# orting/image-feature-extraction

Hardware: AMD Instinct MI355X
Metric: Mvoxels/sec Hessian+eig, 512^3 fp32 3-scale (higher is better)
Workload: dtype f32 storage / f64 line recurrences

## Files before the change

image-feature-extraction_amd/__init__.py:

```python
import ctypes as C
import os

import numpy as np

_HERE = os.path.dirname(os.path.abspath(__file__))
LIB_PATH = os.environ.get("IFE_HIP_LIB") or os.path.join(_HERE, "csrc", "libife_hip.so")

OK, E_ARG, E_SIZE, E_HIP, E_NOMEM, E_STATE = 0, -1, -2, -3, -4, -5
F32, I16, U8, U16 = 0, 1, 2, 3
INTERLEAVED, PLANAR = 0, 1
MEM_HOST, MEM_DEVICE = 0, 1
OPT_TRIG_MODE, OPT_DSCALE_MODE, OPT_PROFILE, OPT_ZCHUNK, OPT_IIR_BLOCK, OPT_IIR_CKPT, OPT_IIR_FMA = 1, 2, 3, 4, 5, 6, 7
OPT_FUSED_DIVIDE = 8
OPT_CONST_LINES = 9
OPT_FEAT_RING = 10
Z_STATE_BYTES = 32
Z_OVERLAP_LO, Z_OVERLAP_HI = 3, 4
NUM_FEATURES = 8
MAX_KERNEL_KINDS = 24
FEATURE_NAMES = ("GaussianBlur", "GradientMagnitude", "Eigenvalue1", "Eigenvalue2",
                 "Eigenvalue3", "LaplacianOfGaussian", "GaussianCurvature", "FrobeniusNorm")

EXPORTS = (
    "ife_abi_version", "ife_ctx_create", "ife_ctx_destroy", "ife_last_error",
    "ife_ctx_set_stream", "ife_ctx_set_option", "ife_ctx_reserve", "ife_ctx_synchronize",
    "ife_eigenvalues", "ife_eigenvalue_features", "ife_hessian3d", "ife_gradient_magnitude",
    "ife_normalized_gaussian_convolution", "ife_differential_normalized_convolution",
    "ife_emphysema_features",
    "ife_emphysema_features_begin", "ife_emphysema_features_fetch", "ife_emphysema_features_end",
    "ife_fd_hessian_features", "ife_fd_gradient_features", "ife_mask_image_f64",
    "ife_get_kernel_times", "ife_reset_kernel_times", "ife_measure_stream",
    "ife_stage_prepare", "ife_stage_recursive_gaussian", "ife_stage_recursive_gaussian_batch",
    "ife_stage_features", "ife_stage_z_ck_bytes", "ife_stage_z_sweep", "ife_stage_z_combine",
    "ife_stage_z_fused", "ife_stage_recursive_gaussian_quotient",
    "ife_multi_create", "ife_multi_destroy", "ife_multi_last_error", "ife_multi_set_option",
    "ife_multi_emphysema_features", "ife_multi_emphysema_features_begin",
    "ife_multi_emphysema_features_fetch", "ife_multi_emphysema_features_end",
    "ife_sort_f32", "ife_equalized_edges_f32", "ife_equalized_edges_f64", "ife_dense_histogram_f32", "ife_roi_histograms", "ife_bag_image",
    "ife_samples_create", "ife_samples_destroy", "ife_samples_count", "ife_samples_clear",
    "ife_samples_add_features", "ife_samples_add_image", "ife_samples_sort",
    "ife_samples_equalized_edges", "ife_samples_read_column",
    "ife_signed_distance_map", "ife_expected_distance",
)


class VolumeDesc(C.Structure):
    _fields_ = [("nx", C.c_int64), ("ny", C.c_int64), ("nz", C.c_int64),
                ("sx", C.c_double), ("sy", C.c_double), ("sz", C.c_double)]
# ... 642 lines not shown
```

image-feature-extraction_amd/csrc/eigen_device.hpp:

```cpp
#pragma once
#include <hip/hip_runtime.h>

namespace ife {

struct Eig3 {
  float e0, e1, e2;
};

template <int TRIG>
__device__ __forceinline__ Eig3 eig3_sym(float A11, float A12, float A13, float A22, float A23,
                                         float A33) {
  Eig3 r;
  float p = A12 * A12 + A13 * A13 + A23 * A23;
  if (p == 0.0f) {
    const float a1 = fabsf(A11), a2 = fabsf(A22), a3 = fabsf(A33);
    if (a1 > a2) {
      if (a1 > a3) {
        r.e0 = A11;
        if (a2 > a3) { r.e1 = A22; r.e2 = A33; }
        else         { r.e1 = A33; r.e2 = A22; }
      } else { r.e0 = A33; r.e1 = A11; r.e2 = A22; }
    } else {
      if (a2 > a3) {
        r.e0 = A22;
// ... 218 lines not shown
    r.e0 = diag ? d0 : r.e0;
    r.e1 = diag ? d1 : r.e1;
    r.e2 = diag ? d2 : r.e2;
  }
  if (__builtin_amdgcn_ballot_w64(unsafe) != 0) {
    const Eig3 g = eig3_sym_generic_call<(TRIG == 2 ? 0 : TRIG)>(A11, A12, A13, A22, A23, A33);
    r.e0 = unsafe ? g.e0 : r.e0;
    r.e1 = unsafe ? g.e1 : r.e1;
    r.e2 = unsafe ? g.e2 : r.e2;
  }
  return r;
}

__device__ __forceinline__ float sqrt_rn_normal(float x) {
  const float s = __builtin_amdgcn_sqrtf(x);
  const float sd = __builtin_bit_cast(float, __builtin_bit_cast(int, s) - 1);
  const float su = __builtin_bit_cast(float, __builtin_bit_cast(int, s) + 1);
  const float ed = fmaf(-sd, s, x);
  const float eu = fmaf(-su, s, x);
  float r = ed <= 0.0f ? sd : s;
  r = eu > 0.0f ? su : r;
  return r;
}
template <int D>
__device__ __forceinline__ float div_by_const_inrange(float x) {
  const float d = (float)D;
  const float y = D == 3 ? 0x1.555556p-2f : 0x1.555556p-3f;
  const float q = x * y;
  const float f = fmaf(fmaf(-d, q, x), y, q);
  return x == 0.0f ? x : f;
}

template <typename KT>
__device__ __forceinline__ Eig3 eig3_sym_fast2(float A11, float A12, float A13, float A22,
                                              float A23, float A33, const KT &K) {
  const float p0 = A12 * A12 + A13 * A13 + A23 * A23;
  const bool diag = p0 == 0.0f;
  const float tr = A11 + A22 + A33;
  const float q = div_by_const_inrange<3>(tr);
  const float d1 = A11 - q, d2 = A22 - q, d3 = A33 - q;
  const float p2 = d1 * d1 + d2 * d2 + d3 * d3 + 2.0f * p0;
  const float atr = fabsf(tr);
  const bool ok = (atr <= 0x1p100f) && (atr >= 0x1p-100f || atr == 0.0f) && (p2 >= 0x1p-100f) &&
                  (p2 <= 0x1p100f);
  const bool unsafe = !diag && !ok;
  const float p = sqrt_rn_normal(div_by_const_inrange<6>(p2));
  const SharedRecip rp = shared_recip(p);
  const float B11 = div_shared(d1, rp), B12 = div_shared(A12, rp), B13 = div_shared(A13, rp);
  const float B22 = div_shared(d2, rp), B23 = div_shared(A23, rp), B33 = div_shared(d3, rp);
  const float r2 = B11 * B22 * B33 + 2.0f * B12 * B13 * B23 - B23 * B23 * B11 -
                   B13 * B13 * B22 - B12 * B12 * B33;
  const float rr = r2 * 0.5f;
  const float twop = 2.0f * p;
  float phi = acos_third_f32(rr);
  phi = rr >= 1.0f ? 0.0f : phi;
  phi = rr <= -1.0f ? (float)(M_PI / 3) : phi;
  float e0 = fmaf(twop, cos_small_f32(phi), q);
  float e2 = fmaf(-twop, cos_small_f32((float)(M_PI / 3) - phi), q);
  float e1 = 3.0f * q - e0 - e2;
  if (fabsf(e0) < fabsf(e2)) { const float t = e0; e0 = e2; e2 = t; }
  if (fabsf(e1) < fabsf(e2)) { const float t = e1; e1 = e2; e2 = t; }
  Eig3 r;
  r.e0 = e0; r.e1 = e1; r.e2 = e2;
  if (__builtin_amdgcn_ballot_w64(diag || unsafe) != 0) {
    const float a1 = fabsf(A11), a2 = fabsf(A22), a3 = fabsf(A33);
    const bool c12 = a1 > a2, c13 = a1 > a3, c23 = a2 > a3;
    const float g0 = c12 ? (c13 ? A11 : A33) : (c23 ? A22 : A33);
    const float g1 = c12 ? (c13 ? (c23 ? A22 : A33) : A11) : (c23 ? (c13 ? A11 : A33) : A22);
    const float g2 = c12 ? (c13 ? (c23 ? A33 : A22) : A22) : (c23 ? (c13 ? A33 : A11) : A11);
    r.e0 = diag ? g0 : r.e0;
    r.e1 = diag ? g1 : r.e1;
    r.e2 = diag ? g2 : r.e2;
    if (__builtin_amdgcn_ballot_w64(unsafe) != 0) {
      const Eig3 g = eig3_sym_generic_call<0>(A11, A12, A13, A22, A23, A33);
      r.e0 = unsafe ? g.e0 : r.e0;
      r.e1 = unsafe ? g.e1 : r.e1;
      r.e2 = unsafe ? g.e2 : r.e2;
    }
  }
  return r;
}

struct EigFeat {
  float f[6];
};

template <int TRIG, typename KT = EigConstImm>
__device__ __forceinline__ EigFeat eig_features(float A11, float A12, float A13, float A22,
                                                float A23, float A33, const KT &K = KT()) {
  Eig3 ev;
  if constexpr (TRIG == 2) ev = eig3_sym_fast2(A11, A12, A13, A22, A23, A33, K);
  else ev = eig3_sym_fast<TRIG>(A11, A12, A13, A22, A23, A33, K);
  EigFeat o;
  o.f[0] = ev.e0;
  o.f[1] = ev.e1;
  o.f[2] = ev.e2;
  o.f[3] = ev.e0 + ev.e1 + ev.e2;
  o.f[4] = ev.e0 * ev.e1 * ev.e2;
  o.f[5] = sqrtf(ev.e0 * ev.e0 + ev.e1 * ev.e1 + ev.e2 * ev.e2);
  return o;
}

}
```

image-feature-extraction_amd/csrc/feature_kernels.hpp:

```cpp
#pragma once
#include <hip/hip_runtime.h>
#include <float.h>
#include <stdint.h>

#include "eigen_device.hpp"

namespace ife {

enum FeatMode {
  FEAT_FEATURES8 = 0,
  FEAT_EIG6 = 1,
  FEAT_HESSIAN6 = 2,
  FEAT_GRADMAG = 3,
  FEAT_SAMPLES8 = 4
};

template <int MODE>
struct FeatNOut {
  static constexpr int value =
      (MODE == FEAT_FEATURES8 || MODE == FEAT_SAMPLES8) ? 8 : (MODE == FEAT_GRADMAG ? 1 : 6);
};

struct FeatGeom {
  int nx, ny, nz;
// ... 26 lines not shown
    if (__builtin_amdgcn_ballot_w64(r.b != 1.0f) == 0) return r.a;
    return r.b != 0.0f ? r.a / r.b : FLT_MAX;
  }
};
struct ValS {
  const float *s;
  struct Raw { float a; };
  __device__ __forceinline__ Raw fetch(int64_t i) const { return Raw{s[i]}; }
  __device__ __forceinline__ float finish(const Raw &r) const { return r.a; }
};
template <typename TI>
struct ValRaw {
  const TI *img;
  struct Raw { TI v; };
  __device__ __forceinline__ Raw fetch(int64_t i) const { return Raw{img[i]}; }
  __device__ __forceinline__ float finish(const Raw &r) const { return (float)r.v; }
};

__device__ __forceinline__ int clampi(int v, int hi) { return v < 0 ? 0 : (v > hi ? hi : v); }

__device__ __forceinline__ double d1(double cm, double cp, float fm, float fp) {
  double s = 0.0;
  s += cm * (double)fm;
  s += cp * (double)fp;
  return s;
}
__device__ __forceinline__ float d2(double ca, double cb, double cc, float fm, float f0,
                                    float fp) {
  double s = 0.0;
  s += ca * (double)fm;
  s += cb * (double)f0;
  s += cc * (double)fp;
  return (float)s;
}

constexpr int FT_TX = 64;
#ifndef IFE_FT_TY
#define IFE_FT_TY 8
#endif
constexpr int FT_TY = IFE_FT_TY;
constexpr int FT_HX = FT_TX + 2;
constexpr int FT_HY = FT_TY + 2;
constexpr int FT_NE = FT_HX * FT_HY;
constexpr int FT_THREADS = FT_TX * FT_TY;
constexpr int FT_NLD = (FT_NE + FT_THREADS - 1) / FT_THREADS;

template <int MODE, bool UNIT, int TRIG, bool KLDS>
__device__ __forceinline__ void feat_point(const float (*tm)[FT_HX], const float (*t0)[FT_HX],
                                           const float (*tp)[FT_HX], int ty, int tx,
                                           const DerivCoef &dc, const double *ktab,
                                           float (&o)[FeatNOut<MODE>::value]) {
  constexpr bool F8 = MODE == FEAT_FEATURES8 || MODE == FEAT_SAMPLES8;
  constexpr bool NEED_H = MODE != FEAT_GRADMAG;
  constexpr bool NEED_G = F8 || MODE == FEAT_GRADMAG;
  const float c = t0[ty + 1][tx + 1];
  const float xm = t0[ty + 1][tx], xp = t0[ty + 1][tx + 2];
  const float ym = t0[ty][tx + 1], yp = t0[ty + 2][tx + 1];
  const float zm = tm[ty + 1][tx + 1], zp = tp[ty + 1][tx + 1];
  float G = 0.0f;
  if (NEED_G) {
    double gx, gy, gz;
    if (UNIT) {
      gx = 0.5 * ((double)xp - (double)xm);
      gy = 0.5 * ((double)yp - (double)ym);
      gz = 0.5 * ((double)zp - (double)zm);
    } else {
      gx = d1(dc.m1[0], dc.p1[0], xm, xp);
      gy = d1(dc.m1[1], dc.p1[1], ym, yp);
      gz = d1(dc.m1[2], dc.p1[2], zm, zp);
    }
    double a = gx * gx;
    a += gy * gy;
    a += gz * gz;
#if defined(IFE_DIAG_NO_GSQRT)
    G = (float)a;
#else
    G = (float)sqrt(a);
#endif
  }
  if constexpr (MODE == FEAT_GRADMAG) {
    o[0] = G;
  } else if (NEED_H) {
    const float cmm = t0[ty][tx], cpm = t0[ty][tx + 2];
    const float cmp = t0[ty + 2][tx], cpp = t0[ty + 2][tx + 2];
    const float zm_xm = tm[ty + 1][tx], zm_xp = tm[ty + 1][tx + 2];
    const float zm_ym = tm[ty][tx + 1], zm_yp = tm[ty + 2][tx + 1];
    const float zp_xm = tp[ty + 1][tx], zp_xp = tp[ty + 1][tx + 2];
    const float zp_ym = tp[ty][tx + 1], zp_yp = tp[ty + 2][tx + 1];
    float dxx, dyy, dzz, dxy, dxz, dyz;
    if (UNIT) {
      const float dx_ym = 0.5f * (cpm - cmm), dx_yp = 0.5f * (cpp - cmp);
      const float dx_zm = 0.5f * (zm_xp - zm_xm), dx_zp = 0.5f * (zp_xp - zp_xm);
      const float dy_zm = 0.5f * (zm_yp - zm_ym), dy_zp = 0.5f * (zp_yp - zp_ym);
      dxy = 0.5f * (dx_yp - dx_ym);
      dxz = 0.5f * (dx_zp - dx_zm);
      dyz = 0.5f * (dy_zp - dy_zm);
      const double cd = (double)c;
      dxx = (float)(fma(-2.0, cd, (double)xm) + (double)xp);
      dyy = (float)(fma(-2.0, cd, (double)ym) + (double)yp);
      dzz = (float)(fma(-2.0, cd, (double)zm) + (double)zp);
    } else {
      const float dx_ym = (float)d1(dc.m1[0], dc.p1[0], cmm, cpm);
      const float dx_yp = (float)d1(dc.m1[0], dc.p1[0], cmp, cpp);
      const float dx_zm = (float)d1(dc.m1[0], dc.p1[0], zm_xm, zm_xp);
      const float dx_zp = (float)d1(dc.m1[0], dc.p1[0], zp_xm, zp_xp);
      const float dy_zm = (float)d1(dc.m1[1], dc.p1[1], zm_ym, zm_yp);
      const float dy_zp = (float)d1(dc.m1[1], dc.p1[1], zp_ym, zp_yp);
      dxy = (float)d1(dc.m1[1], dc.p1[1], dx_ym, dx_yp);
      dxz = (float)d1(dc.m1[2], dc.p1[2], dx_zm, dx_zp);
      dyz = (float)d1(dc.m1[2], dc.p1[2], dy_zm, dy_zp);
// ... 253 lines not shown
  r.w = 0x00020000u;
  return r;
}
__device__ __forceinline__ void ft_dma_dword(ft_u32x4 rsrc, uint32_t voff, uint32_t lds_addr) {
  uint32_t keep;
  asm volatile(
      "s_mov_b32 %0, m0\n\t"
      "s_mov_b32 m0, %3\n\t"
      "s_nop 0\n\t"
      "buffer_load_dword %1, %2, 0 offen lds\n\t"
      "s_mov_b32 m0, %0"
      : "=&s"(keep)
      : "v"(voff), "s"(rsrc), "s"(lds_addr)
      : "memory");
}
__device__ __forceinline__ void ft_wait_vmcnt(int n) {
#define IFE_W(k) case k: asm volatile("s_waitcnt vmcnt(" #k ")" ::: "memory"); break;
  switch (n) {
    IFE_W(0) IFE_W(1) IFE_W(2) IFE_W(3) IFE_W(4) IFE_W(5) IFE_W(6) IFE_W(7) IFE_W(8) IFE_W(9)
    IFE_W(10) IFE_W(11) IFE_W(12) IFE_W(13) IFE_W(14) IFE_W(15) IFE_W(16) IFE_W(17) IFE_W(18)
    IFE_W(19) IFE_W(20) IFE_W(21) IFE_W(22) IFE_W(23) IFE_W(24) IFE_W(25) IFE_W(26) IFE_W(27)
    IFE_W(28) IFE_W(29) IFE_W(30) IFE_W(31) IFE_W(32) IFE_W(33) IFE_W(34) IFE_W(35) IFE_W(36)
    default: asm volatile("s_waitcnt vmcnt(0)" ::: "memory"); break;
  }
#undef IFE_W
}
__device__ __forceinline__ void ft_lds_barrier() {
  asm volatile("s_waitcnt lgkmcnt(0)\n\ts_barrier" ::: "memory");
}
#ifndef IFE_FT_NT_AUX
#define IFE_FT_NT_AUX (IFE_FT_NT ? 2 : 0)
#endif

template <int MODE, bool UNIT, int TRIG, bool PLANAR, typename TM>
__global__ __launch_bounds__(FT_THREADS, IFE_FT_WAVES(MODE, UNIT, TRIG)) void features_ring_kernel(
    const float *__restrict__ val, const TM *__restrict__ mask, float *__restrict__ out, FeatGeom g,
    DerivCoef dc) {
  static_assert(sizeof(TM) <= 2, "mask tiles of wider types do not fit the slot");
  using rsrc_t = __amdgpu_buffer_rsrc_t;
  constexpr int NOUT = FeatNOut<MODE>::value;
  constexpr bool F8 = MODE == FEAT_FEATURES8 || MODE == FEAT_SAMPLES8;
  constexpr bool SAMPLES = MODE == FEAT_SAMPLES8;
  static_assert(!SAMPLES || PLANAR, "sample columns are written through the planar store");
  constexpr bool KLDS = (F8 || MODE == FEAT_EIG6) && IFE_FT_KLDS && TRIG != 2;
  constexpr bool XPOSE = !PLANAR && (NOUT == 8 || NOUT == 6);
  constexpr int XW = NOUT == 8 ? 4 : 2;
  constexpr int XN = XPOSE ? NOUT / XW : 1;
  constexpr int NST = XPOSE ? XN : NOUT;
  constexpr int MT_DW = FT_TY * FT_TX * (int)sizeof(TM) / 4;
  constexpr int MT_DWROW = FT_TX * (int)sizeof(TM) / 4;
  constexpr int MPIECES = MT_DW / 64;

  __shared__ __attribute__((aligned(16))) uint32_t ring[FR_NS * FR_SLOT_DW];
  __shared__ float xstrip[XPOSE ? FT_THREADS / 64 : 1][XPOSE ? 64 * NOUT : 1];
  __shared__ double ktab[KLDS ? EK_COUNT : 1];
  if (KLDS) eig_const_fill(ktab);

  const int tid = threadIdx.x;
  const int tx = tid & 63;
  const int w = (int)__builtin_amdgcn_readfirstlane((uint32_t)tid >> 6);
  int bx, by, bz;
  {
    const uint32_t nb = (uint32_t)g.gx * (uint32_t)g.gy * (uint32_t)g.gz;
    const uint32_t lin = blockIdx.x;
    const uint32_t per = nb / 8u, rem = nb % 8u;
    const uint32_t c = lin % 8u, i = lin / 8u;
    const uint32_t t = c * per + (c < rem ? c : rem) + i;
    bx = (int)(t % (uint32_t)g.gx);
    by = (int)((t / (uint32_t)g.gx) % (uint32_t)g.gy);
    bz = (int)(t / ((uint32_t)g.gx * (uint32_t)g.gy));
  }
  const int x = bx * FT_TX + tx, y = by * FT_TY + w;
  const int z0 = bz * g.zchunk;
  const int z1 = min(z0 + g.zchunk, g.nz);
  const bool has_mask = mask != nullptr;
  const int row_valid = y < g.ny ? min(FT_TX, g.nx - bx * FT_TX) : 0;

  auto val_off = [&](int e) -> uint32_t {
    if (e >= FT_NE) e = 0;
    const int ey = e / FT_HX, ex = e % FT_HX;
    return 4u * ((uint32_t)clampi(bx * FT_TX - 1 + ex, g.nx - 1) +
                 (uint32_t)g.nx * (uint32_t)clampi(by * FT_TY - 1 + ey, g.ny - 1));
  };
  const uint32_t offA = val_off(tid);
  const bool b_val = w < FR_VPIECES - 8;
  const bool b_mask = !b_val && has_mask && (w - (FR_VPIECES - 8)) < MPIECES;
  const int n_dma = 1 + ((b_val || b_mask) ? 1 : 0);
  uint32_t offB = 0;
  if (b_val) {
    offB = val_off(FT_THREADS + tid);
  } else if (b_mask) {
    const int d = (w - (FR_VPIECES - 8)) * 64 + tx;
    int mx = bx * FT_TX + (d % MT_DWROW) * (4 / (int)sizeof(TM));
    int my = by * FT_TY + d / MT_DWROW;
    if (mx >= g.nx || my >= g.ny) { mx = bx * FT_TX; my = by * FT_TY; }
    offB = (uint32_t)sizeof(TM) * ((uint32_t)mx + (uint32_t)g.nx * (uint32_t)my);
  }
  const uint32_t lds0 = (uint32_t)(uintptr_t)(__attribute__((address_space(3))) void *)ring;
  const uint32_t dstA = (uint32_t)w * 256u;
  const uint32_t dstB = b_val ? (uint32_t)(8 + w) * 256u
                              : (uint32_t)FR_VDW * 4u + (uint32_t)(w - (FR_VPIECES - 8)) * 256u;
  auto slot_of = [&](int p) { return (uint32_t)(p - (z0 - 1)) & (uint32_t)(FR_NS - 1); };
  auto request = [&](int p) {
    const uint32_t sb = lds0 + slot_of(p) * (uint32_t)(FR_SLOT_DW * 4);
// ... 226 lines not shown
```

image-feature-extraction_amd/csrc/ife_capi.hip:

```cpp
#include "../../include/ife_hip.h"

#include <hip/hip_runtime.h>

#include <algorithm>
#include <cmath>
#include <cstdarg>
#include <cstdio>
#include <cstdlib>
#include <cstring>
#include <map>
#include <new>
#include <string>
#include <tuple>
#include <type_traits>
#include <vector>

#include "feature_kernels.hpp"
#include "iir_types.hpp"
#include "stats_kernels.hpp"
#include "distance_kernels.hpp"
#define IFE_IIR_NS iir_exact
#define IFE_IIR_FMA 0
#include "iir_kernels.inc"
#undef IFE_IIR_NS
// ... 38 lines not shown
  KK_IIR_Z = 0,
  KK_IIR_X,
  KK_IIR_Y,
  KK_ZSLAB_SWEEP,
  KK_ZSLAB_COMBINE,
  KK_FEATURES,
  KK_EIG_BATCH,
  KK_DIVIDE,
  KK_MASK,
  KK_PREP,
  KK_SORT_HIST,
  KK_SORT_SCAN,
  KK_SORT_SCATTER,
  KK_GATHER,
  KK_EDGES,
  KK_HIST,
  KK_EDT_X,
  KK_EDT_Y,
  KK_EDT_Z,
  KK_EDT_REDUCE,
  KK_COUNT
};
static_assert(KK_COUNT <= IFE_MAX_KERNEL_KINDS, "ife_get_kernel_times callers size their arrays by IFE_MAX_KERNEL_KINDS");
const char *kKindNames[KK_COUNT] = {"iir_z", "iir_x", "iir_y", "zslab_sweep", "zslab_combine", "features", "eig_batch",
                                    "divide", "mask_f64", "prep", "sort_hist", "sort_scan",
                                    "sort_scatter", "gather", "edges", "dense_histogram", "edt_x", "edt_y",
                                    "edt_z", "edt_reduce"};

struct DevBuf {
  void *p = nullptr;
  size_t cap = 0;
};
constexpr int IFE_MAX_SLOTS = 3;

struct ProfRec {
  int kind;
  hipEvent_t a, b;
};

thread_local std::string g_create_error;

}

struct ife_ctx {
  int device = 0;
  hipStream_t stream = nullptr;
  std::string err;
  int trig_mode = 2;
  int dscale_mode = 0;
  int profile = 0;
  int zchunk = 64;
  int iir_block = 0;
  int iir_fma = 0;
  int iir_ckpt = 2;
  int fused_divide = 1;
  int const_lines = 1;
  int feat_ring = 1;
  std::map<std::tuple<double, double, int64_t>, uint32_t> const_flags;
  DevBuf fld[IFE_MAX_SLOTS][4];
  DevBuf pre[2];
  DevBuf ck_y[IIR_MAX_JOBS], ck_x[IIR_MAX_JOBS];
  DevBuf st_img, st_mask, st_aux, st_out;
  DevBuf edt_g, edt_i, edt_d2, edt_part;
  DevBuf sc_out;
  std::vector<hipEvent_t> sc_done;
  hipStream_t sc_copy = nullptr;
  size_t sc_scale_bytes = 0;
  std::vector<hipEvent_t> *scale_events = nullptr;
  std::vector<ProfRec> prof;
  std::vector<hipEvent_t> ev_pool;
  double acc_ms[KK_COUNT] = {0};
  int64_t acc_n[KK_COUNT] = {0};
};

namespace {

int fail(ife_ctx *ctx, int code, const char *fmt, ...) {
  char buf[512];
  va_list ap;
  va_start(ap, fmt);
  vsnprintf(buf, sizeof buf, fmt, ap);
  va_end(ap);
  if (ctx) ctx->err = buf;
  else g_create_error = buf;
  return code;
}

#define IFE_HIP(ctx, call)                                                                  \
  do {                                                                                      \
    hipError_t e_ = (call);                                                                 \
// ... 454 lines not shown
    for (int k = 0; k < nscales; ++k)
      for (int f = 0; f < nf; ++f, ++j) {
        in[j] = from_source ? (f == 0 ? src_num : src_den)
                            : (const float *)ctx->fld[k][2 * f + src_idx].p;
        out[j] = (float *)ctx->fld[k][2 * f + dst_idx].p;
      }
  };
  fill(0, 0, true);
  rc = launch_iir(ctx, v, 2, nj, in, out, sg);
  fill(0, 1, false);
  if (!rc) rc = launch_iir(ctx, v, 0, nj, in, out, sg);
  if (nf == 2 && ctx->fused_divide && ctx->iir_ckpt == 2) {
    const float *n1[IIR_MAX_JOBS], *d1[IIR_MAX_JOBS];
    float *o1[IIR_MAX_JOBS];
    double s1[IIR_MAX_JOBS];
    for (int k = 0; k < nscales; ++k) {
      n1[k] = (const float *)ctx->fld[k][1].p;
      d1[k] = (const float *)ctx->fld[k][3].p;
      o1[k] = (float *)ctx->fld[k][0].p;
      s1[k] = sigmas[k];
    }
    if (!rc) rc = launch_iir(ctx, v, 1, nscales, n1, o1, s1, 1, nullptr, d1);
    return rc;
  }
  fill(1, 0, false);
  if (!rc) rc = launch_iir(ctx, v, 1, nj, in, out, sg);
  return rc;
}
bool slots_hold_quotient(const ife_ctx *ctx, bool has_den) {
  return has_den && ctx->fused_divide && ctx->iir_ckpt == 2;
}

template <int MODE, typename VAL, typename TM>
int launch_features(ife_ctx *ctx, VAL val, const TM *mask, float *out,
                    const ife_volume_desc *v, int layout, int halo_lo = 0, int halo_hi = 0,
                    const uint32_t *seg_base = nullptr, int64_t col_stride = 0,
                    int64_t col_offset = 0) {
  if constexpr (std::is_same<VAL, ValSmooth>::value) {
    if (val.den == nullptr)
      return launch_features<MODE>(ctx, ValS{val.num}, mask, out, v, layout, halo_lo, halo_hi,
                                   seg_base, col_stride, col_offset);
  }
  FeatGeom g;
  g.seg_base = seg_base;
  g.col_offset = col_offset;
  g.nx = (int)v->nx; g.ny = (int)v->ny; g.nz = (int)v->nz;
  g.zchunk = ctx->zchunk;
  g.plane = v->nx * v->ny;
  g.nvox = MODE == FEAT_SAMPLES8 ? col_stride : g.plane * v->nz;
  g.zoff = halo_lo ? 1 : 0;
  g.zc_hi = (int)v->nz + g.zoff + (halo_hi ? 1 : 0) - 1;
  const DerivCoef dc = deriv_coeffs(v, ctx->dscale_mode);
  g.gx = (int)((v->nx + FT_TX - 1) / FT_TX);
  g.gy = (int)((v->ny + FT_TY - 1) / FT_TY);
  g.gz = (int)((v->nz + g.zchunk - 1) / g.zchunk);
  const int64_t nblocks = (int64_t)g.gx * g.gy * g.gz;
  if (nblocks > 0x7fffffff) return fail(ctx, IFE_E_SIZE, "volume too large for the feature kernel grid");
  {
    constexpr int nout = FeatNOut<MODE>::value;
    const uintptr_t need = layout == IFE_PLANAR ? 4 : (nout == 8 ? 16 : nout == 6 ? 8 : 4);
    if (reinterpret_cast<uintptr_t>(out) % need)
      return fail(ctx, IFE_E_ARG, "output pointer must be aligned to %d bytes for this layout", (int)need);
  }
  dim3 grid((unsigned)nblocks, 1, 1);
  ProfScope ps(ctx, KK_FEATURES);
  const bool unit = v->sx == 1.0 && v->sy == 1.0 && v->sz == 1.0;
  const int planar = layout == IFE_PLANAR ? 1 : 0;
  constexpr bool has_eig = MODE == FEAT_FEATURES8 || MODE == FEAT_EIG6 || MODE == FEAT_SAMPLES8;
  constexpr bool ring_types = (std::is_same<VAL, ValS>::value || std::is_same<VAL, ValRaw<float>>::value) &&
                              sizeof(TM) <= 2;
  bool ring = false;
  const float *ring_src = nullptr;
  if constexpr (ring_types) {
    if constexpr (std::is_same<VAL, ValS>::value) ring_src = val.s;
    else ring_src = val.img;
    const int64_t row_bytes = v->nx * (int64_t)sizeof(TM), plane_bytes = g.plane * (int64_t)sizeof(TM);
    ring = ctx->feat_ring && g.plane < ((int64_t)1 << 30) && reinterpret_cast<uintptr_t>(ring_src) % 4 == 0 &&
           (mask == nullptr ||
            (row_bytes % 4 == 0 && plane_bytes % 4 == 0 && reinterpret_cast<uintptr_t>(mask) % 4 == 0));
  }
  auto launch = [&](auto UNIT, auto TRIG, auto PL) {
    constexpr bool U = decltype(UNIT)::value != 0, P = decltype(PL)::value != 0;
    constexpr int T = decltype(TRIG)::value;
    if constexpr (ring_types) {
      if (ring) {
        hipLaunchKernelGGL((features_ring_kernel<MODE, U, T, P, TM>), grid, dim3(FT_THREADS), 0, ctx->stream,
                           ring_src, mask, out, g, dc);
        return;
      }
    }
    hipLaunchKernelGGL((features_kernel<MODE, U, T, P, VAL, TM>), grid, dim3(FT_THREADS), 0, ctx->stream, val,
                       mask, out, g, dc);
  };
  with_const<1, 0>(unit, [&](auto UNIT) {
    auto with_trig = [&](auto TRIG) {
      if constexpr (MODE == FEAT_SAMPLES8) launch(UNIT, TRIG, std::true_type{});
      else with_const<1, 0>(planar, [&](auto PL) { launch(UNIT, TRIG, PL); });
    };
    if constexpr (has_eig) with_const<1, 2, 0>(ctx->trig_mode, with_trig);
    else with_trig(std::integral_constant<int, 0>{});
  });
  IFE_HIP(ctx, hipGetLastError());
  return IFE_OK;
}

size_t dtype_size(int dt) {
  switch (dt) {
    case IFE_F32: return 4;
    case IFE_I16: return 2;
    case IFE_U8: return 1;
    case IFE_U16: return 2;
  }
  return 0;
}

int check_mem(ife_ctx *ctx, int mem) {
  if (mem != IFE_MEM_HOST && mem != IFE_MEM_DEVICE) return fail(ctx, IFE_E_ARG, "bad mem %d", mem);
  return IFE_OK;
}
int check_layout_mem(ife_ctx *ctx, int layout, int mem) {
  if (layout != IFE_INTERLEAVED && layout != IFE_PLANAR)
    return fail(ctx, IFE_E_ARG, "bad layout %d", layout);
  return check_mem(ctx, mem);
}
int check_image_dtype(ife_ctx *ctx, int dt) {
  if (dt != IFE_F32 && dt != IFE_I16) return fail(ctx, IFE_E_ARG, "image dtype must be IFE_F32 or IFE_I16");
  return IFE_OK;
}
int check_mask_dtype(ife_ctx *ctx, const void *mask, int dt, bool may_be_null) {
  if (!mask) return may_be_null ? IFE_OK : fail(ctx, IFE_E_ARG, "null pointer");
  if (dt != IFE_U8 && dt != IFE_U16) return fail(ctx, IFE_E_ARG, "mask dtype must be IFE_U8 or IFE_U16");
  return IFE_OK;
}
int check_sigma(ife_ctx *ctx, double sigma) {
  if (!(sigma > 0.0)) return fail(ctx, IFE_E_ARG, "sigma must be positive");
  return IFE_OK;
// ... 56 lines not shown
  IFE_HIP(ctx, hipSetDevice(ctx->device));
  (void)hipGetLastError();
  return IFE_OK;
}

}

struct SampleSink {
  const uint8_t *code;
  const uint32_t *seg_base;
  float *columns;
  int64_t stride, offset;
};

template <typename TI, typename TM>
static int emphysema_typed(ife_ctx *ctx, const TI *img, const TM *msk, const ife_volume_desc *vol,
                           const float *sigmas, int n_sigmas, float *dout, int layout,
                           const SampleSink *sink = nullptr) {
  const size_t n = (size_t)(vol->nx * vol->ny * vol->nz);
  float *tc = (float *)ctx->pre[0].p, *cf = (float *)ctx->pre[1].p;
  const float *src_num;
  if (msk == nullptr && std::is_same<TI, float>::value) {
    src_num = reinterpret_cast<const float *>(img);
  } else {
    int rc = launch_prep<TI, TM>(ctx, img, msk, tc, msk ? cf : nullptr, (int64_t)n);
    if (rc) return rc;
    src_num = tc;
  }
  for (int s0 = 0; s0 < n_sigmas; s0 += IFE_MAX_SLOTS) {
    const int ns = std::min(IFE_MAX_SLOTS, n_sigmas - s0);
    double sg[IFE_MAX_SLOTS];
    for (int k = 0; k < ns; ++k) sg[k] = (double)sigmas[s0 + k];
    int rc = smooth_group(ctx, src_num, msk ? cf : nullptr, vol, sg, ns);
    for (int k = 0; k < ns && !rc; ++k) {
      const bool q = slots_hold_quotient(ctx, msk != nullptr);
      const ValSmooth vs{(const float *)ctx->fld[k][0].p, msk && !q ? (const float *)ctx->fld[k][2].p : nullptr};
      if (sink)
        rc = launch_features<FEAT_SAMPLES8>(ctx, vs, sink->code,
                                            sink->columns + (size_t)(s0 + k) * IFE_NUM_FEATURES * sink->stride,
                                            vol, IFE_PLANAR, 0, 0, sink->seg_base, sink->stride, sink->offset);
      else
        rc = launch_features<FEAT_FEATURES8>(ctx, vs, msk, dout + (size_t)(s0 + k) * n * IFE_NUM_FEATURES, vol,
                                             layout);
      if (!rc && ctx->scale_events) {
        hipEvent_t e;
        IFE_HIP(ctx, hipEventCreateWithFlags(&e, hipEventDisableTiming));
        ctx->scale_events->push_back(e);
        IFE_HIP(ctx, hipEventRecord(e, ctx->stream));
      }
    }
    if (rc) return rc;
  }
  return IFE_OK;
}

static int emphysema_check(ife_ctx *ctx, const void *image, int image_dtype, const void *mask, int mask_dtype,
                           const ife_volume_desc *vol, const float *sigmas, int n_sigmas, bool have_out,
                           int layout, int mem) {
  int rc;
  if ((rc = check_vol(ctx, vol, true))) return rc;
  if ((rc = check_layout_mem(ctx, layout, mem))) return rc;
  if (!image || !have_out || !sigmas) return fail(ctx, IFE_E_ARG, "null pointer");
  if ((rc = check_sigmas(ctx, sigmas, n_sigmas))) return rc;
  if ((rc = check_image_dtype(ctx, image_dtype))) return rc;
  return check_mask_dtype(ctx, mask, mask_dtype, true);
}

static int emphysema_staged(ife_ctx *ctx, int mem, const void *image, int image_dtype, const void *mask,
                            int mask_dtype, const ife_volume_desc *vol, const float *sigmas, int n_sigmas,
                            float *dout, int layout, hipEvent_t *uploaded = nullptr) {
  const size_t n = (size_t)(vol->nx * vol->ny * vol->nz);
  const void *dI, *dM;
  int rc;
  if ((rc = stage_in(ctx, mem, image, n * dtype_size(image_dtype), ctx->st_img, &dI))) return rc;
  if ((rc = stage_in(ctx, mem, mask, n * (mask ? dtype_size(mask_dtype) : 0), ctx->st_mask, &dM))) {
    if (uploaded) (void)hipStreamSynchronize(ctx->stream);
// ... 77 lines not shown
  if (!ctx) return IFE_E_ARG;
  switch (option) {
    case IFE_OPT_TRIG_MODE:
      if (value < 0 || value > 2) return fail(ctx, IFE_E_ARG, "trig mode must be 0, 1 or 2");
      ctx->trig_mode = value;
      return IFE_OK;
    case IFE_OPT_DSCALE_MODE:
      if (value != 0 && value != 1) return fail(ctx, IFE_E_ARG, "dscale mode must be 0 or 1");
      ctx->dscale_mode = value;
      return IFE_OK;
    case IFE_OPT_PROFILE:
      ctx->profile = value ? 1 : 0;
      return IFE_OK;
    case IFE_OPT_ZCHUNK:
      if (value < 1) return fail(ctx, IFE_E_ARG, "zchunk must be >= 1");
      ctx->zchunk = value;
      return IFE_OK;
    case IFE_OPT_IIR_FMA:
      ctx->iir_fma = value ? 1 : 0;
      return IFE_OK;
    case IFE_OPT_IIR_CKPT:
      if (value != 1 && value != 2) return fail(ctx, IFE_E_ARG, "iir checkpoint stride must be 1 or 2");
      ctx->iir_ckpt = value;
      return IFE_OK;
    case IFE_OPT_CONST_LINES:
      ctx->const_lines = value ? 1 : 0;
      return IFE_OK;
    case IFE_OPT_FUSED_DIVIDE:
      ctx->fused_divide = value ? 1 : 0;
      return IFE_OK;
    case IFE_OPT_FEAT_RING:
      ctx->feat_ring = value ? 1 : 0;
      return IFE_OK;
    case IFE_OPT_IIR_BLOCK:
      if (value != 0 && value != 8 && value != 10 && value != 12 && value != 16)
        return fail(ctx, IFE_E_ARG, "iir block must be 0 (per axis), 8, 10, 12 (strided axes only; x keeps 16) or 16");
      ctx->iir_block = value;
      return IFE_OK;
  }
  return fail(ctx, IFE_E_ARG, "unknown option %d", option);
}

int ife_ctx_reserve(ife_ctx *ctx, const ife_volume_desc *vol) {
  int rc = bind(ctx);
  if (rc) return rc;
  rc = check_vol(ctx, vol, false);
  if (rc) return rc;
  const size_t nb = (size_t)(vol->nx * vol->ny * vol->nz) * sizeof(float);
  rc = ensure_slots(ctx, vol, IFE_MAX_SLOTS);
  for (int i = 0; i < 2 && !rc; ++i) rc = ensure(ctx, ctx->pre[i], nb);
  if (!rc) rc = ensure_ck(ctx, vol, 2 * IFE_MAX_SLOTS);
  return rc;
}

int ife_ctx_synchronize(ife_ctx *ctx) {
  int rc = bind(ctx);
  if (rc) return rc;
  IFE_HIP(ctx, hipStreamSynchronize(ctx->stream));
  return IFE_OK;
}

static int eig_batch(ife_ctx *ctx, const float *A6, int64_t n, float *outv, int mem, int nout) {
  int rc = bind(ctx);
  if (rc) return rc;
  if (n < 0 || (n > 0 && (!A6 || !outv))) return fail(ctx, IFE_E_ARG, "null pointer");
  if ((rc = check_mem(ctx, mem))) return rc;
// ... 460 lines not shown
```

include/ife_hip.h:

```cpp
#ifndef IFE_HIP_H
#define IFE_HIP_H

#include <stddef.h>
#include <stdint.h>

#ifdef __cplusplus
extern "C" {
#endif

#define IFE_ABI_VERSION 1

typedef struct ife_ctx ife_ctx;

typedef enum {
  IFE_OK = 0,
  IFE_E_ARG = -1,
  IFE_E_SIZE = -2,
  IFE_E_HIP = -3,
  IFE_E_NOMEM = -4,
  IFE_E_STATE = -5
} ife_status;

typedef enum { IFE_F32 = 0, IFE_I16 = 1, IFE_U8 = 2, IFE_U16 = 3 } ife_dtype;
typedef enum { IFE_INTERLEAVED = 0, IFE_PLANAR = 1 } ife_layout;
typedef enum { IFE_MEM_HOST = 0, IFE_MEM_DEVICE = 1 } ife_mem;

typedef enum {
  IFE_OPT_TRIG_MODE = 1,
  IFE_OPT_DSCALE_MODE = 2,
  IFE_OPT_PROFILE = 3,
  IFE_OPT_ZCHUNK = 4,
  IFE_OPT_IIR_BLOCK = 5,
  IFE_OPT_IIR_CKPT = 6,
  IFE_OPT_IIR_FMA = 7,
  IFE_OPT_FUSED_DIVIDE = 8,
  IFE_OPT_CONST_LINES = 9,
  IFE_OPT_FEAT_RING = 10
} ife_option;

typedef struct {
  int64_t nx, ny, nz;
  double sx, sy, sz;
} ife_volume_desc;

#define IFE_NUM_FEATURES 8
#define IFE_FEATURE_NAMES                                                              \
  {"GaussianBlur", "GradientMagnitude", "Eigenvalue1", "Eigenvalue2", "Eigenvalue3",   \
   "LaplacianOfGaussian", "GaussianCurvature", "FrobeniusNorm"}


int ife_abi_version(void);
int ife_ctx_create(int device, ife_ctx **ctx);
void ife_ctx_destroy(ife_ctx *ctx);
const char *ife_last_error(const ife_ctx *ctx);
int ife_ctx_set_stream(ife_ctx *ctx, void *hip_stream);
int ife_ctx_set_option(ife_ctx *ctx, int option, int value);
int ife_ctx_reserve(ife_ctx *ctx, const ife_volume_desc *vol);
int ife_ctx_synchronize(ife_ctx *ctx);


int ife_eigenvalues(ife_ctx *ctx, const float *A6, int64_t n, float *ev3, int mem);
int ife_eigenvalue_features(ife_ctx *ctx, const float *A6, int64_t n, float *f6, int mem);


int ife_hessian3d(ife_ctx *ctx, const float *image, const ife_volume_desc *vol, float *out6,
                  int layout, int mem);

int ife_gradient_magnitude(ife_ctx *ctx, const float *image, const ife_volume_desc *vol,
                           float *out, int mem);

// ... 143 lines not shown
```

Baseline: 45730.

## Batch per-scale feature launches into one ring kernel and speed up sqrt paths

New measurement: 45680. About the same (-0.1%).

```diff
diff --git a/image-feature-extraction_amd/__init__.py b/image-feature-extraction_amd/__init__.py
--- a/image-feature-extraction_amd/__init__.py
+++ b/image-feature-extraction_amd/__init__.py
@@ -14,6 +14,7 @@
 OPT_FUSED_DIVIDE = 8
 OPT_CONST_LINES = 9
 OPT_FEAT_RING = 10
+OPT_FEAT_BATCH = 11
 Z_STATE_BYTES = 32
 Z_OVERLAP_LO, Z_OVERLAP_HI = 3, 4
 NUM_FEATURES = 8
diff --git a/image-feature-extraction_amd/csrc/eigen_device.hpp b/image-feature-extraction_amd/csrc/eigen_device.hpp
--- a/image-feature-extraction_amd/csrc/eigen_device.hpp
+++ b/image-feature-extraction_amd/csrc/eigen_device.hpp
@@ -274,10 +274,11 @@
 }
 
 template <typename KT>
-__device__ __forceinline__ Eig3 eig3_sym_fast2(float A11, float A12, float A13, float A22,
-                                              float A23, float A33, const KT &K) {
+__device__ __forceinline__ Eig3 eig3_fast2_common(float A11, float A12, float A13, float A22,
+                                                 float A23, float A33, const KT &K, bool &diag,
+                                                 bool &unsafe) {
   const float p0 = A12 * A12 + A13 * A13 + A23 * A23;
-  const bool diag = p0 == 0.0f;
+  diag = p0 == 0.0f;
   const float tr = A11 + A22 + A33;
   const float q = div_by_const_inrange<3>(tr);
   const float d1 = A11 - q, d2 = A22 - q, d3 = A33 - q;
@@ -285,7 +286,7 @@
   const float atr = fabsf(tr);
   const bool ok = (atr <= 0x1p100f) && (atr >= 0x1p-100f || atr == 0.0f) && (p2 >= 0x1p-100f) &&
                   (p2 <= 0x1p100f);
-  const bool unsafe = !diag && !ok;
+  unsafe = !diag && !ok;
   const float p = sqrt_rn_normal(div_by_const_inrange<6>(p2));
   const SharedRecip rp = shared_recip(p);
   const float B11 = div_shared(d1, rp), B12 = div_shared(A12, rp), B13 = div_shared(A13, rp);
@@ -304,22 +305,33 @@
   if (fabsf(e1) < fabsf(e2)) { const float t = e1; e1 = e2; e2 = t; }
   Eig3 r;
   r.e0 = e0; r.e1 = e1; r.e2 = e2;
-  if (__builtin_amdgcn_ballot_w64(diag || unsafe) != 0) {
-    const float a1 = fabsf(A11), a2 = fabsf(A22), a3 = fabsf(A33);
-    const bool c12 = a1 > a2, c13 = a1 > a3, c23 = a2 > a3;
-    const float g0 = c12 ? (c13 ? A11 : A33) : (c23 ? A22 : A33);
-    const float g1 = c12 ? (c13 ? (c23 ? A22 : A33) : A11) : (c23 ? (c13 ? A11 : A33) : A22);
-    const float g2 = c12 ? (c13 ? (c23 ? A33 : A22) : A22) : (c23 ? (c13 ? A33 : A11) : A11);
-    r.e0 = diag ? g0 : r.e0;
-    r.e1 = diag ? g1 : r.e1;
-    r.e2 = diag ? g2 : r.e2;
-    if (__builtin_amdgcn_ballot_w64(unsafe) != 0) {
-      const Eig3 g = eig3_sym_generic_call<0>(A11, A12, A13, A22, A23, A33);
-      r.e0 = unsafe ? g.e0 : r.e0;
-      r.e1 = unsafe ? g.e1 : r.e1;
-      r.e2 = unsafe ? g.e2 : r.e2;
-    }
-  }
+  return r;
+}
+__device__ __forceinline__ void eig3_fast2_rare(float A11, float A12, float A13, float A22,
+                                                float A23, float A33, bool diag, bool unsafe,
+                                                Eig3 &r) {
+  const float a1 = fabsf(A11), a2 = fabsf(A22), a3 = fabsf(A33);
+  const bool c12 = a1 > a2, c13 = a1 > a3, c23 = a2 > a3;
+  const float g0 = c12 ? (c13 ? A11 : A33) : (c23 ? A22 : A33);
+  const float g1 = c12 ? (c13 ? (c23 ? A22 : A33) : A11) : (c23 ? (c13 ? A11 : A33) : A22);
+  const float g2 = c12 ? (c13 ? (c23 ? A33 : A22) : A22) : (c23 ? (c13 ? A33 : A11) : A11);
+  r.e0 = diag ? g0 : r.e0;
+  r.e1 = diag ? g1 : r.e1;
+  r.e2 = diag ? g2 : r.e2;
+  if (__builtin_amdgcn_ballot_w64(unsafe) != 0) {
+    const Eig3 g = eig3_sym_generic_call<0>(A11, A12, A13, A22, A23, A33);
+    r.e0 = unsafe ? g.e0 : r.e0;
+    r.e1 = unsafe ? g.e1 : r.e1;
+    r.e2 = unsafe ? g.e2 : r.e2;
+  }
+}
+template <typename KT>
+__device__ __forceinline__ Eig3 eig3_sym_fast2(float A11, float A12, float A13, float A22,
+                                              float A23, float A33, const KT &K) {
+  bool diag, unsafe;
+  Eig3 r = eig3_fast2_common(A11, A12, A13, A22, A23, A33, K, diag, unsafe);
+  if (__builtin_amdgcn_ballot_w64(diag || unsafe) != 0)
+    eig3_fast2_rare(A11, A12, A13, A22, A23, A33, diag, unsafe, r);
   return r;
 }
 
@@ -331,15 +343,26 @@
 __device__ __forceinline__ EigFeat eig_features(float A11, float A12, float A13, float A22,
                                                 float A23, float A33, const KT &K = KT()) {
   Eig3 ev;
-  if constexpr (TRIG == 2) ev = eig3_sym_fast2(A11, A12, A13, A22, A23, A33, K);
+  bool diag = false, unsafe = false;
+  if constexpr (TRIG == 2) ev = eig3_fast2_common(A11, A12, A13, A22, A23, A33, K, diag, unsafe);
   else ev = eig3_sym_fast<TRIG>(A11, A12, A13, A22, A23, A33, K);
+  float ss = ev.e0 * ev.e0 + ev.e1 * ev.e1 + ev.e2 * ev.e2;
+  const bool wide = !(ss >= 0x1p-100f && ss <= 0x1p100f);
+  float fro = sqrt_rn_normal(ss);
+  if (__builtin_amdgcn_ballot_w64(diag || unsafe || wide) != 0) {
+    if constexpr (TRIG == 2) {
+      eig3_fast2_rare(A11, A12, A13, A22, A23, A33, diag, unsafe, ev);
+      ss = ev.e0 * ev.e0 + ev.e1 * ev.e1 + ev.e2 * ev.e2;
+    }
+    fro = sqrtf(ss);
+  }
   EigFeat o;
   o.f[0] = ev.e0;
   o.f[1] = ev.e1;
   o.f[2] = ev.e2;
   o.f[3] = ev.e0 + ev.e1 + ev.e2;
   o.f[4] = ev.e0 * ev.e1 * ev.e2;
-  o.f[5] = sqrtf(ev.e0 * ev.e0 + ev.e1 * ev.e1 + ev.e2 * ev.e2);
+  o.f[5] = fro;
   return o;
 }
 
diff --git a/image-feature-extraction_amd/csrc/feature_kernels.hpp b/image-feature-extraction_amd/csrc/feature_kernels.hpp
--- a/image-feature-extraction_amd/csrc/feature_kernels.hpp
+++ b/image-feature-extraction_amd/csrc/feature_kernels.hpp
@@ -82,6 +82,30 @@
   s += cb * (double)f0;
   s += cc * (double)fp;
   return (float)s;
+}
+
+constexpr uint32_t GR_MARGIN = 4;
+template <bool QUARTER>
+__device__ __forceinline__ float grad_root(double a) {
+  const double y0 = __builtin_amdgcn_rsq(a);
+  double g = a * y0, h = 0.5 * y0;
+  const double e = fma(-h, g, 0.5);
+  g = fma(g, e, g);
+  h = fma(h, e, h);
+  g = fma(fma(-g, g, a), h, g);
+  const uint32_t glo = (uint32_t)__builtin_bit_cast(uint64_t, g);
+  const uint32_t ahi = (uint32_t)(__builtin_bit_cast(uint64_t, a) >> 32);
+  const bool near = ((glo - (0x10000000u - GR_MARGIN)) & 0x1fffffffu) <= 2u * GR_MARGIN;
+  const bool outside = (ahi - 0x30500000u) >= (0x4fd00000u - 0x30500000u);
+  float G = (float)g;
+  if (QUARTER) G *= 0.5f;
+  const bool rare = near || outside;
+  if (__builtin_amdgcn_ballot_w64(rare) != 0) {
+    float L = 0.0f;
+    if (__builtin_amdgcn_ballot_w64(rare && a != 0.0) != 0) L = (float)sqrt(QUARTER ? 0.25 * a : a);
+    G = rare ? L : G;
+  }
+  return G;
 }
 
 constexpr int FT_TX = 64;
@@ -111,9 +135,9 @@
   if (NEED_G) {
     double gx, gy, gz;
     if (UNIT) {
-      gx = 0.5 * ((double)xp - (double)xm);
-      gy = 0.5 * ((double)yp - (double)ym);
-      gz = 0.5 * ((double)zp - (double)zm);
+      gx = (double)xp - (double)xm;
+      gy = (double)yp - (double)ym;
+      gz = (double)zp - (double)zm;
     } else {
       gx = d1(dc.m1[0], dc.p1[0], xm, xp);
       gy = d1(dc.m1[1], dc.p1[1], ym, yp);
@@ -125,7 +149,7 @@
 #if defined(IFE_DIAG_NO_GSQRT)
     G = (float)a;
 #else
-    G = (float)sqrt(a);
+    G = grad_root<UNIT>(a);
 #endif
   }
   if constexpr (MODE == FEAT_GRADMAG) {
@@ -445,10 +469,16 @@
 #define IFE_FT_NT_AUX (IFE_FT_NT ? 2 : 0)
 #endif
 
+constexpr int FEAT_MAX_BATCH = 3;
+struct FeatBatch {
+  const float *val[FEAT_MAX_BATCH];
+  float *out[FEAT_MAX_BATCH];
+  int n;
+};
+
 template <int MODE, bool UNIT, int TRIG, bool PLANAR, typename TM>
 __global__ __launch_bounds__(FT_THREADS, IFE_FT_WAVES(MODE, UNIT, TRIG)) void features_ring_kernel(
-    const float *__restrict__ val, const TM *__restrict__ mask, float *__restrict__ out, FeatGeom g,
-    DerivCoef dc) {
+    FeatBatch batch, const TM *__restrict__ mask, FeatGeom g, DerivCoef dc) {
   static_assert(sizeof(TM) <= 2, "mask tiles of wider types do not fit the slot");
   using rsrc_t = __amdgpu_buffer_rsrc_t;
   constexpr int NOUT = FeatNOut<MODE>::value;
@@ -473,16 +503,22 @@
   const int tx = tid & 63;
   const int w = (int)__builtin_amdgcn_readfirstlane((uint32_t)tid >> 6);
   int bx, by, bz;
+  uint32_t sc;
   {
-    const uint32_t nb = (uint32_t)g.gx * (uint32_t)g.gy * (uint32_t)g.gz;
+    const uint32_t ns = (uint32_t)batch.n;
+    const uint32_t nb = (uint32_t)g.gx * (uint32_t)g.gy * (uint32_t)g.gz * ns;
     const uint32_t lin = blockIdx.x;
     const uint32_t per = nb / 8u, rem = nb % 8u;
     const uint32_t c = lin % 8u, i = lin / 8u;
-    const uint32_t t = c * per + (c < rem ? c : rem) + i;
+    const uint32_t ts = c * per + (c < rem ? c : rem) + i;
+    const uint32_t t = ts / ns;
+    sc = ts % ns;
     bx = (int)(t % (uint32_t)g.gx);
     by = (int)((t / (uint32_t)g.gx) % (uint32_t)g.gy);
     bz = (int)(t / ((uint32_t)g.gx * (uint32_t)g.gy));
   }
+  const float *__restrict__ val = sc == 0 ? batch.val[0] : (sc == 1 ? batch.val[1] : batch.val[2]);
+  float *__restrict__ out = sc == 0 ? batch.out[0] : (sc == 1 ? batch.out[1] : batch.out[2]);
   const int x = bx * FT_TX + tx, y = by * FT_TY + w;
   const int z0 = bz * g.zchunk;
   const int z1 = min(z0 + g.zchunk, g.nz);
diff --git a/image-feature-extraction_amd/csrc/ife_capi.hip b/image-feature-extraction_amd/csrc/ife_capi.hip
--- a/image-feature-extraction_amd/csrc/ife_capi.hip
+++ b/image-feature-extraction_amd/csrc/ife_capi.hip
@@ -94,6 +94,7 @@
   size_t cap = 0;
 };
 constexpr int IFE_MAX_SLOTS = 3;
+static_assert(IFE_MAX_SLOTS <= FEAT_MAX_BATCH, "a slot group must fit one batched feature launch");
 
 struct ProfRec {
   int kind;
@@ -118,6 +119,7 @@
   int fused_divide = 1;
   int const_lines = 1;
   int feat_ring = 1;
+  int feat_batch = 1;
   std::map<std::tuple<double, double, int64_t>, uint32_t> const_flags;
   DevBuf fld[IFE_MAX_SLOTS][4];
   DevBuf pre[2];
@@ -638,14 +640,20 @@
 }
 
 template <int MODE, typename VAL, typename TM>
-int launch_features(ife_ctx *ctx, VAL val, const TM *mask, float *out,
-                    const ife_volume_desc *v, int layout, int halo_lo = 0, int halo_hi = 0,
-                    const uint32_t *seg_base = nullptr, int64_t col_stride = 0,
-                    int64_t col_offset = 0) {
+int launch_features_n(ife_ctx *ctx, const VAL *vals, int nsc, const TM *mask, float *const *outs,
+                      const ife_volume_desc *v, int layout, int halo_lo = 0, int halo_hi = 0,
+                      const uint32_t *seg_base = nullptr, int64_t col_stride = 0,
+                      int64_t col_offset = 0) {
+  if (nsc < 1 || nsc > FEAT_MAX_BATCH) return fail(ctx, IFE_E_ARG, "feature batch of %d scales", nsc);
   if constexpr (std::is_same<VAL, ValSmooth>::value) {
-    if (val.den == nullptr)
-      return launch_features<MODE>(ctx, ValS{val.num}, mask, out, v, layout, halo_lo, halo_hi,
-                                   seg_base, col_stride, col_offset);
+    bool single = true;
+    for (int k = 0; k < nsc; ++k) single = single && vals[k].den == nullptr;
+    if (single) {
+      ValS vs[FEAT_MAX_BATCH];
+      for (int k = 0; k < nsc; ++k) vs[k] = ValS{vals[k].num};
+      return launch_features_n<MODE>(ctx, vs, nsc, mask, outs, v, layout, halo_lo, halo_hi, seg_base,
+                                     col_stride, col_offset);
+    }
   }
   FeatGeom g;
   g.seg_base = seg_base;
@@ -661,42 +669,50 @@
   g.gy = (int)((v->ny + FT_TY - 1) / FT_TY);
   g.gz = (int)((v->nz + g.zchunk - 1) / g.zchunk);
   const int64_t nblocks = (int64_t)g.gx * g.gy * g.gz;
-  if (nblocks > 0x7fffffff) return fail(ctx, IFE_E_SIZE, "volume too large for the feature kernel grid");
+  if (nblocks * nsc > 0x7fffffff) return fail(ctx, IFE_E_SIZE, "volume too large for the feature kernel grid");
   {
     constexpr int nout = FeatNOut<MODE>::value;
     const uintptr_t need = layout == IFE_PLANAR ? 4 : (nout == 8 ? 16 : nout == 6 ? 8 : 4);
-    if (reinterpret_cast<uintptr_t>(out) % need)
-      return fail(ctx, IFE_E_ARG, "output pointer must be aligned to %d bytes for this layout", (int)need);
-  }
-  dim3 grid((unsigned)nblocks, 1, 1);
-  ProfScope ps(ctx, KK_FEATURES);
+    for (int k = 0; k < nsc; ++k)
+      if (reinterpret_cast<uintptr_t>(outs[k]) % need)
+        return fail(ctx, IFE_E_ARG, "output pointer must be aligned to %d bytes for this layout", (int)need);
+  }
   const bool unit = v->sx == 1.0 && v->sy == 1.0 && v->sz == 1.0;
   const int planar = layout == IFE_PLANAR ? 1 : 0;
   constexpr bool has_eig = MODE == FEAT_FEATURES8 || MODE == FEAT_EIG6 || MODE == FEAT_SAMPLES8;
   constexpr bool ring_types = (std::is_same<VAL, ValS>::value || std::is_same<VAL, ValRaw<float>>::value) &&
                               sizeof(TM) <= 2;
   bool ring = false;
-  const float *ring_src = nullptr;
+  FeatBatch batch = {};
   if constexpr (ring_types) {
-    if constexpr (std::is_same<VAL, ValS>::value) ring_src = val.s;
-    else ring_src = val.img;
     const int64_t row_bytes = v->nx * (int64_t)sizeof(TM), plane_bytes = g.plane * (int64_t)sizeof(TM);
-    ring = ctx->feat_ring && g.plane < ((int64_t)1 << 30) && reinterpret_cast<uintptr_t>(ring_src) % 4 == 0 &&
+    ring = ctx->feat_ring && g.plane < ((int64_t)1 << 30) &&
            (mask == nullptr ||
             (row_bytes % 4 == 0 && plane_bytes % 4 == 0 && reinterpret_cast<uintptr_t>(mask) % 4 == 0));
+    batch.n = nsc;
+    for (int k = 0; k < nsc; ++k) {
+      if constexpr (std::is_same<VAL, ValS>::value) batch.val[k] = vals[k].s;
+      else batch.val[k] = vals[k].img;
+      batch.out[k] = outs[k];
+      ring = ring && reinterpret_cast<uintptr_t>(batch.val[k]) % 4 == 0;
+    }
   }
   auto launch = [&](auto UNIT, auto TRIG, auto PL) {
     constexpr bool U = decltype(UNIT)::value != 0, P = decltype(PL)::value != 0;
     constexpr int T = decltype(TRIG)::value;
     if constexpr (ring_types) {
       if (ring) {
-        hipLaunchKernelGGL((features_ring_kernel<MODE, U, T, P, TM>), grid, dim3(FT_THREADS), 0, ctx->stream,
-                           ring_src, mask, out, g, dc);
+        ProfScope ps(ctx, KK_FEATURES);
+        hipLaunchKernelGGL((features_ring_kernel<MODE, U, T, P, TM>), dim3((unsigned)(nblocks * nsc)),
+                           dim3(FT_THREADS), 0, ctx->stream, batch, mask, g, dc);
         return;
       }
     }
-    hipLaunchKernelGGL((features_kernel<MODE, U, T, P, VAL, TM>), grid, dim3(FT_THREADS), 0, ctx->stream, val,
-                       mask, out, g, dc);
+    for (int k = 0; k < nsc; ++k) {
+      ProfScope ps(ctx, KK_FEATURES);
+      hipLaunchKernelGGL((features_kernel<MODE, U, T, P, VAL, TM>), dim3((unsigned)nblocks), dim3(FT_THREADS), 0,
+                         ctx->stream, vals[k], mask, outs[k], g, dc);
+    }
   };
   with_const<1, 0>(unit, [&](auto UNIT) {
     auto with_trig = [&](auto TRIG) {
@@ -708,6 +724,14 @@
   });
   IFE_HIP(ctx, hipGetLastError());
   return IFE_OK;
+}
+template <int MODE, typename VAL, typename TM>
+int launch_features(ife_ctx *ctx, VAL val, const TM *mask, float *out,
+                    const ife_volume_desc *v, int layout, int halo_lo = 0, int halo_hi = 0,
+                    const uint32_t *seg_base = nullptr, int64_t col_stride = 0,
+                    int64_t col_offset = 0) {
+  return launch_features_n<MODE>(ctx, &val, 1, mask, &out, v, layout, halo_lo, halo_hi, seg_base, col_stride,
+                                 col_offset);
 }
 
 size_t dtype_size(int dt) {
@@ -830,16 +854,25 @@
     double sg[IFE_MAX_SLOTS];
     for (int k = 0; k < ns; ++k) sg[k] = (double)sigmas[s0 + k];
     int rc = smooth_group(ctx, src_num, msk ? cf : nullptr, vol, sg, ns);
+    const bool q = slots_hold_quotient(ctx, msk != nullptr);
+    ValSmooth vs[IFE_MAX_SLOTS];
+    float *outs[IFE_MAX_SLOTS];
+    for (int k = 0; k < ns; ++k) {
+      vs[k] = ValSmooth{(const float *)ctx->fld[k][0].p, msk && !q ? (const float *)ctx->fld[k][2].p : nullptr};
+      outs[k] = sink ? sink->columns + (size_t)(s0 + k) * IFE_NUM_FEATURES * sink->stride
+                     : dout + (size_t)(s0 + k) * n * IFE_NUM_FEATURES;
+    }
+    if (!rc && !sink && !ctx->scale_events && ctx->feat_batch) {
+      rc = launch_features_n<FEAT_FEATURES8>(ctx, vs, ns, msk, outs, vol, layout);
+      if (rc) return rc;
+      continue;
+    }
     for (int k = 0; k < ns && !rc; ++k) {
-      const bool q = slots_hold_quotient(ctx, msk != nullptr);
-      const ValSmooth vs{(const float *)ctx->fld[k][0].p, msk && !q ? (const float *)ctx->fld[k][2].p : nullptr};
       if (sink)
-        rc = launch_features<FEAT_SAMPLES8>(ctx, vs, sink->code,
-                                            sink->columns + (size_t)(s0 + k) * IFE_NUM_FEATURES * sink->stride,
-                                            vol, IFE_PLANAR, 0, 0, sink->seg_base, sink->stride, sink->offset);
+        rc = launch_features<FEAT_SAMPLES8>(ctx, vs[k], sink->code, outs[k], vol, IFE_PLANAR, 0, 0, sink->seg_base,
+                                            sink->stride, sink->offset);
       else
-        rc = launch_features<FEAT_FEATURES8>(ctx, vs, msk, dout + (size_t)(s0 + k) * n * IFE_NUM_FEATURES, vol,
-                                             layout);
+        rc = launch_features<FEAT_FEATURES8>(ctx, vs[k], msk, outs[k], vol, layout);
       if (!rc && ctx->scale_events) {
         hipEvent_t e;
         IFE_HIP(ctx, hipEventCreateWithFlags(&e, hipEventDisableTiming));
@@ -983,6 +1016,9 @@
     case IFE_OPT_FEAT_RING:
       ctx->feat_ring = value ? 1 : 0;
       return IFE_OK;
+    case IFE_OPT_FEAT_BATCH:
+      ctx->feat_batch = value ? 1 : 0;
+      return IFE_OK;
     case IFE_OPT_IIR_BLOCK:
       if (value != 0 && value != 8 && value != 10 && value != 12 && value != 16)
         return fail(ctx, IFE_E_ARG, "iir block must be 0 (per axis), 8, 10, 12 (strided axes only; x keeps 16) or 16");
diff --git a/include/ife_hip.h b/include/ife_hip.h
--- a/include/ife_hip.h
+++ b/include/ife_hip.h
@@ -35,7 +35,8 @@
   IFE_OPT_IIR_FMA = 7,
   IFE_OPT_FUSED_DIVIDE = 8,
   IFE_OPT_CONST_LINES = 9,
-  IFE_OPT_FEAT_RING = 10
+  IFE_OPT_FEAT_RING = 10,
+  IFE_OPT_FEAT_BATCH = 11
 } ife_option;
 
 typedef struct {
```
